# daijifeng001/MNC

Measured on NVIDIA H100. Metric: images/sec VGG16 MNC 5-stage @600x1000, 300 RoIs, higher is better.
Workload: dtype f16+2xf8 (fp16 main product + two e4m3 correction products on wgmma, fp32 accumulate, fp32-parity; conv1_1, K = 27: bf16x3)

## Files before the change

### mnc_b200/csrc/igemm_tc.cu

```cuda
#include <cuda.h>
#include <cuda_bf16.h>
#include <cuda_fp16.h>
#include <cuda_fp8.h>
#include <cuda_runtime.h>
#include <cstdint>
#include <cstdio>

#include "mnc_b200.h"
#include "ptx.cuh"
#include "tri.cuh"
#include "launch_util.h"

namespace mnc {

struct IgemmArgs {
  int batch, H, W;
  int Cin, Cout;
  int taps;
  int tiles_h, tiles_w, tiles_n;
  int k_steps;
  int split_k;
  int relu;
  int out_mode;
  const float* bias;
  __nv_bfloat16* out_hi;
  __nv_bfloat16* out_lo;
  uint8_t* out_x;
  float* out_f32;
  float acc_scale;
  float out_scale;
  unsigned int* amax;
  long long out_pix_stride;
  int out_ch_offset;
  long long split_stride;
  int vec_ok;
  int tma_store;
};

constexpr int kBlockM = 128;
constexpr int kBlockK = 64;
constexpr int kSmemMax = 227 * 1024;

constexpr int kXchgStride = 33;
constexpr int kXchgBytes = 2 * 128 * kXchgStride * 4;
constexpr int kStagingBytes = 2 * 2 * 128 * 64;
constexpr int kBarrierBytes = 1024;

template <int BN>
struct IgemmCfg {
  static constexpr int kABytes = kBlockM * kBlockK * 2;
  static constexpr int kBBytes = BN * kBlockK * 2;
  static constexpr int kStageBytes = 2 * kABytes + 2 * kBBytes;
  static constexpr int kFixedBytes = 1024  + kBarrierBytes + kXchgBytes + kStagingBytes;
  static constexpr int kStagesRaw = (kSmemMax - kFixedBytes) / kStageBytes;
  static constexpr int kStages = kStagesRaw > 8 ? 8 : kStagesRaw;
  static constexpr int kSmemBytes = kStages * kStageBytes + kFixedBytes;
  static_assert(kStages >= 2, "the ring needs two stages");
};

struct Tile {
  int img, h0, w0, n0, ks;
  int kb, kn, kstride;
};

__device__ __forceinline__ Tile decode_tile(const IgemmArgs& p, int t, int TH, int TW, int BN) {
  const int per_img = p.tiles_h * p.tiles_w;
  const int spatial = p.batch * per_img;
  const int sp = t % spatial;
  const int rest = t / spatial;
  const int nt = rest % p.tiles_n;
  Tile tl;
  tl.ks = rest / p.tiles_n;
  tl.img = sp / per_img;
  const int r = sp % per_img;
  tl.h0 = (r / p.tiles_w) * TH;
  tl.w0 = (r % p.tiles_w) * TW;
  tl.n0 = nt * BN;
  tl.kb = tl.ks;
  tl.kstride = p.split_k;
  tl.kn = (p.k_steps - tl.ks + p.split_k - 1) / p.split_k;
  return tl;
}


struct EpiState {
  int chunk_ctr;
  float amx;
};

template <int TH, int TW, int BN>
__device__ __forceinline__ void epilogue_tile(const IgemmArgs& p, const CUtensorMap* tm_o_hi_p,
                                              const CUtensorMap* tm_o_lo_p,
                                              const CUtensorMap* tm_o_x_p, float* xchg,
                                              uint8_t* staging, float (&acc)[BN / 64][32],
                                              const Tile& tl, int grp, EpiState& st) {
  const int tid = threadIdx.x & 127;
  const int lane = threadIdx.x & 31;
  constexpr int NBUF = 1;
  const int lead = 128 + grp * 128;
  const int row = tid;
  int& chunk_ctr = st.chunk_ctr;
  float& amx = st.amx;
  const float asc = p.acc_scale;
  const int img = tl.img, h0 = tl.h0, w0 = tl.w0, n0 = tl.n0, ks = tl.ks;
  const int h = h0 + row / TW;
  const int w = w0 + row % TW;
  const bool valid = (h < p.H) && (w < p.W);
  const long long pix = (static_cast<long long>(img) * p.H + h) * p.W + w;
  const int frow = grp * 64 + (tid >> 5) * 16 + (lane >> 2);
  const int fcol = (lane & 3) * 2;
#pragma unroll
  for (int nb = 0; nb < BN / 64; ++nb) {
    const int c0 = nb * 64 + grp * 32;
    uint32_t r[32];
    {
#pragma unroll
      for (int j = 0; j < 8; ++j) {
        const int col = j * 8 + fcol;
        float* d0 = xchg + ((col >> 5) * 128 + frow) * kXchgStride + (col & 31);
        d0[0] = acc[nb][4 * j];
        d0[1] = acc[nb][4 * j + 1];
        d0[8 * kXchgStride] = acc[nb][4 * j + 2];
        d0[8 * kXchgStride + 1] = acc[nb][4 * j + 3];
      }
      ptx::named_bar_sync(1, 256);
      const float* s0 = xchg + (grp * 128 + row) * kXchgStride;
#pragma unroll
      for (int j = 0; j < 32; ++j) r[j] = __float_as_uint(s0[j]);
      ptx::named_bar_sync(2, 256);
    }
      const int ch0 = n0 + c0;
      if (p.out_mode == 3) continue;
      if (p.out_mode == 2 || p.out_mode == 5) {
        const bool odd_x = (lane & 1) != 0;
        const bool odd_y = ((lane / TW) & 1) != 0;
        const int part = (odd_x ? 2 : 0) | (odd_y ? 1 : 0);
        const int hl = (row / TW) & ~1;
        const int wl = (row % TW) & ~1;
        float x[32];
#pragma unroll
        for (int j = 0; j < 32; ++j) x[j] = __uint_as_float(r[j]);
        if (!__all_sync(0xffffffffu, valid)) {
#pragma unroll
          for (int j = 0; j < 32; ++j) x[j] = valid ? x[j] : -3.402823466e+38f;
        }
        float y[16], m[8];
#pragma unroll
        for (int j = 0; j < 16; ++j) {
          const float keep = odd_x ? x[j + 16] : x[j];
          const float send = odd_x ? x[j] : x[j + 16];
          y[j] = fmaxf(keep, __shfl_xor_sync(0xffffffffu, send, 1));
        }
#pragma unroll
        for (int j = 0; j < 8; ++j) {
          const float keep = odd_y ? y[j + 8] : y[j];
          const float send = odd_y ? y[j] : y[j + 8];
          m[j] = fmaxf(keep, __shfl_xor_sync(0xffffffffu, send, TW));
        }
        const int hp = (h0 + hl) >> 1;
        const int wp = (w0 + wl) >> 1;
        const int Ho = (p.H + 1) >> 1, Wo = (p.W + 1) >> 1;
        const int chp = ch0 + part * 8;
        if (hp < Ho && wp < Wo && (h0 + hl) < p.H && (w0 + wl) < p.W &&
            chp < p.Cout) {
          const long long ppix = (static_cast<long long>(img) * Ho + hp) * Wo + wp;
          const long long poff = ppix * p.out_pix_stride + p.out_ch_offset + chp;
          float bv[8];
          if (p.bias != nullptr && chp + 8 <= p.Cout && (reinterpret_cast<uintptr_t>(p.bias + chp) & 15) == 0) {
            const float4 b0 = __ldg(reinterpret_cast<const float4*>(p.bias + chp));
            const float4 b1 = __ldg(reinterpret_cast<const float4*>(p.bias + chp) + 1);
            bv[0] = b0.x, bv[1] = b0.y, bv[2] = b0.z, bv[3] = b0.w;
            bv[4] = b1.x, bv[5] = b1.y, bv[6] = b1.z, bv[7] = b1.w;
          } else {
#pragma unroll
            for (int j = 0; j < 8; ++j)
              bv[j] = (p.bias != nullptr && chp + j < p.Cout) ? __ldg(p.bias + chp + j) : 0.f;
          }
#pragma unroll
          for (int j = 0; j < 8; ++j) {
            m[j] = m[j] * asc + bv[j];
            if (p.relu) m[j] = fmaxf(m[j], 0.f);
            if (chp + j < p.Cout) amx = fmaxf(amx, fabsf(m[j]));
          }
          if (p.out_mode == 5) {
            uint32_t hw[4], lw[2], cw[2];
#pragma unroll
            for (int e = 0; e < 4; ++e) {
              const Tri2 tr = tri_pack2(m[2 * e], m[2 * e + 1], p.out_scale);
              hw[e] = tr.h;
              if (e & 1) {
                lw[e >> 1] |= static_cast<uint32_t>(tr.l) << 16;
                cw[e >> 1] |= static_cast<uint32_t>(tr.c) << 16;
              } else {
                lw[e >> 1] = tr.l;
                cw[e >> 1] = tr.c;
              }
            }
            *reinterpret_cast<uint4*>(reinterpret_cast<__half*>(p.out_hi) + poff) =
                make_uint4(hw[0], hw[1], hw[2], hw[3]);
            *reinterpret_cast<uint2*>(reinterpret_cast<uint8_t*>(p.out_lo) + poff) = make_uint2(lw[0], lw[1]);
            *reinterpret_cast<uint2*>(p.out_x + poff) = make_uint2(cw[0], cw[1]);
            continue;
          }
          __nv_bfloat16* ph = p.out_hi + poff;
          __nv_bfloat16* pl = p.out_lo + poff;
          uint32_t hw[4], lw[4];
#pragma unroll
          for (int e = 0; e < 4; ++e) {
            const float x0 = m[2 * e], x1 = m[2 * e + 1];
            const __nv_bfloat16 h0b = __float2bfloat16_rn(x0);
            const __nv_bfloat16 h1b = __float2bfloat16_rn(x1);
            const __nv_bfloat16 l0b = __float2bfloat16_rn(x0 - __bfloat162float(h0b));
            const __nv_bfloat16 l1b = __float2bfloat16_rn(x1 - __bfloat162float(h1b));
            hw[e] = static_cast<uint32_t>(__bfloat16_as_ushort(h0b)) |
                    (static_cast<uint32_t>(__bfloat16_as_ushort(h1b)) << 16);
            lw[e] = static_cast<uint32_t>(__bfloat16_as_ushort(l0b)) |
                    (static_cast<uint32_t>(__bfloat16_as_ushort(l1b)) << 16);
          }
          *reinterpret_cast<uint4*>(ph) = make_uint4(hw[0], hw[1], hw[2], hw[3]);
          *reinterpret_cast<uint4*>(pl) = make_uint4(lw[0], lw[1], lw[2], lw[3]);
        }
      } else if (p.tma_store) {
        const bool tri = (p.out_mode == 4);
        const int buf = chunk_ctr % NBUF;
        uint8_t* sb = staging + (grp * NBUF + buf) * (2 * 128 * 64);
        if (threadIdx.x == lead) ptx::tma_store_wait_read<NBUF - 1>();
        ptx::named_bar_sync(3 + grp, 128);
        if (ch0 < p.Cout) {
          float bv[32];
          if (p.bias != nullptr && ch0 + 32 <= p.Cout &&
              (reinterpret_cast<uintptr_t>(p.bias + ch0) & 15) == 0) {
#pragma unroll
            for (int j4 = 0; j4 < 8; ++j4) {
              const float4 b4 = __ldg(reinterpret_cast<const float4*>(p.bias + ch0) + j4);
              bv[4 * j4] = b4.x;
              bv[4 * j4 + 1] = b4.y;
              bv[4 * j4 + 2] = b4.z;
              bv[4 * j4 + 3] = b4.w;
            }
          } else {
#pragma unroll
            for (int j = 0; j < 32; ++j)
              bv[j] = (p.bias != nullptr && ch0 + j < p.Cout) ? __ldg(p.bias + ch0 + j) : 0.f;
          }
          float mx = 0.f;
#pragma unroll
          for (int g = 0; g < 4; ++g) {
            uint32_t hw[4], lw[4];
#pragma unroll
            for (int e = 0; e < 4; ++e) {
              float x0 = __uint_as_float(r[g * 8 + 2 * e]) * asc + bv[g * 8 + 2 * e];
              float x1 = __uint_as_float(r[g * 8 + 2 * e + 1]) * asc + bv[g * 8 + 2 * e + 1];
              if (p.relu) {
                x0 = fmaxf(x0, 0.f);
                x1 = fmaxf(x1, 0.f);
              }
              mx = fmaxf(mx, fmaxf(fabsf(x0), fabsf(x1)));
              if (tri) {
                const Tri2 tr = tri_pack2(x0, x1, p.out_scale);
                hw[e] = tr.h;
                if (e & 1) {
                  lw[e >> 1] |= static_cast<uint32_t>(tr.l) << 16;
                  lw[2 + (e >> 1)] |= static_cast<uint32_t>(tr.c) << 16;
                } else {
                  lw[e >> 1] = tr.l;
                  lw[2 + (e >> 1)] = tr.c;
                }
              } else {
                const __nv_bfloat162 hp = __floats2bfloat162_rn(x0, x1);
                const uint32_t hbits = *reinterpret_cast<const uint32_t*>(&hp);
                const float f0 = __uint_as_float(hbits << 16);
                const float f1 = __uint_as_float(hbits & 0xffff0000u);
                const __nv_bfloat162 lp = __floats2bfloat162_rn(x0 - f0, x1 - f1);
                hw[e] = hbits;
                lw[e] = *reinterpret_cast<const uint32_t*>(&lp);
              }
            }
            const int off = row * 64 + ((g ^ ((row >> 1) & 3)) << 4);
            *reinterpret_cast<uint4*>(sb + off) = make_uint4(hw[0], hw[1], hw[2], hw[3]);
            if (tri) {
              *reinterpret_cast<uint2*>(sb + 128 * 64 + row * 32 + g * 8) = make_uint2(lw[0], lw[1]);
              *reinterpret_cast<uint2*>(sb + 128 * 96 + row * 32 + g * 8) = make_uint2(lw[2], lw[3]);
            } else {
              *reinterpret_cast<uint4*>(sb + 128 * 64 + off) = make_uint4(lw[0], lw[1], lw[2], lw[3]);
            }
          }
          if (valid) amx = fmaxf(amx, mx);
        }
        ptx::fence_proxy_async();
        ptx::named_bar_sync(3 + grp, 128);
        if (threadIdx.x == lead && ch0 < p.Cout) {
          ptx::tma_store_4d(tm_o_hi_p, sb, ch0, w0, h0, img);
          ptx::tma_store_4d(tm_o_lo_p, sb + 128 * 64, ch0, w0, h0, img);
          if (tri) ptx::tma_store_4d(tm_o_x_p, sb + 128 * 96, ch0, w0, h0, img);
          ptx::tma_store_commit();
        }
        ++chunk_ctr;
      } else if (valid && ch0 < p.Cout) {
        float v[32];
#pragma unroll
        for (int j = 0; j < 32; ++j) {
          float x = __uint_as_float(r[j]) * asc;
          if (p.bias != nullptr && ch0 + j < p.Cout) x += __ldg(p.bias + ch0 + j);
          if (p.relu) x = fmaxf(x, 0.f);
          v[j] = x;
          if (ch0 + j < p.Cout) amx = fmaxf(amx, fabsf(x));
        }
        const bool fullchunk = (ch0 + 32 <= p.Cout) && p.vec_ok;
        if (p.out_mode == 0) {
          __nv_bfloat16* ph = p.out_hi + pix * p.out_pix_stride + p.out_ch_offset + ch0;
          __nv_bfloat16* pl = p.out_lo + pix * p.out_pix_stride + p.out_ch_offset + ch0;
          if (fullchunk) {
#pragma unroll
            for (int g = 0; g < 4; ++g) {
              uint32_t hw[4], lw[4];
#pragma unroll
              for (int e = 0; e < 4; ++e) {
                const float x0 = v[g * 8 + 2 * e], x1 = v[g * 8 + 2 * e + 1];
                const __nv_bfloat16 h0b = __float2bfloat16_rn(x0);
                const __nv_bfloat16 h1b = __float2bfloat16_rn(x1);
                const __nv_bfloat16 l0b = __float2bfloat16_rn(x0 - __bfloat162float(h0b));
                const __nv_bfloat16 l1b = __float2bfloat16_rn(x1 - __bfloat162float(h1b));
                hw[e] = static_cast<uint32_t>(__bfloat16_as_ushort(h0b)) |
                        (static_cast<uint32_t>(__bfloat16_as_ushort(h1b)) << 16);
                lw[e] = static_cast<uint32_t>(__bfloat16_as_ushort(l0b)) |
                        (static_cast<uint32_t>(__bfloat16_as_ushort(l1b)) << 16);
              }
              *reinterpret_cast<uint4*>(ph + g * 8) = make_uint4(hw[0], hw[1], hw[2], hw[3]);
              *reinterpret_cast<uint4*>(pl + g * 8) = make_uint4(lw[0], lw[1], lw[2], lw[3]);
            }
          } else {
            for (int j = 0; j < 32 && ch0 + j < p.Cout; ++j) {
              const __nv_bfloat16 hb = __float2bfloat16_rn(v[j]);
              ph[j] = hb;
              pl[j] = __float2bfloat16_rn(v[j] - __bfloat162float(hb));
            }
          }
        } else {
          float* po = p.out_f32 + ks * p.split_stride + pix * p.out_pix_stride +
                      p.out_ch_offset + ch0;
          if (fullchunk) {
#pragma unroll
            for (int g = 0; g < 8; ++g)
              *reinterpret_cast<float4*>(po + g * 4) =
                  make_float4(v[g * 4], v[g * 4 + 1], v[g * 4 + 2], v[g * 4 + 3]);
          } else {
            for (int j = 0; j < 32 && ch0 + j < p.Cout; ++j) po[j] = v[j];
          }
        }
      }
  }
}

__device__ __forceinline__ void epilogue_finish(const IgemmArgs& p, int grp, const EpiState& st) {
  if (threadIdx.x == 128 + grp * 128) ptx::tma_store_wait_read<0>();
  if (p.amax != nullptr) {
    float amx = st.amx;
#pragma unroll
    for (int o = 16; o > 0; o >>= 1) amx = fmaxf(amx, __shfl_xor_sync(0xffffffffu, amx, o));
    if ((threadIdx.x & 31) == 0 && amx > 0.f) atomicMax(p.amax, __float_as_uint(amx));
  }
}

template <int TH, int TW, int BN, int PM>
__global__ void __launch_bounds__(384, 1)
igemm_tc_kernel(const __grid_constant__ CUtensorMap tm_a_hi, const __grid_constant__ CUtensorMap tm_a_lo,
                const __grid_constant__ CUtensorMap tm_a_x,
                const __grid_constant__ CUtensorMap tm_b_hi, const __grid_constant__ CUtensorMap tm_b_lo,
                const __grid_constant__ CUtensorMap tm_b_x,
                const __grid_constant__ CUtensorMap tm_o_hi, const __grid_constant__ CUtensorMap tm_o_lo,
                const __grid_constant__ CUtensorMap tm_o_x,
                const IgemmArgs p) {
  static_assert(TH * TW == kBlockM, "pixel tile must have 128 rows");
  using Cfg = IgemmCfg<BN>;
  constexpr int kStages = Cfg::kStages;
  constexpr int kABytes = Cfg::kABytes;
  constexpr int kBBytes = Cfg::kBBytes;
  constexpr int NB = BN / 64;

  extern __shared__ uint8_t smem_raw[];
  uint8_t* smem = reinterpret_cast<uint8_t*>((reinterpret_cast<uintptr_t>(smem_raw) + 1023) &
                                             ~static_cast<uintptr_t>(1023));
  uint64_t* full_bar = reinterpret_cast<uint64_t*>(smem + kStages * Cfg::kStageBytes);
  uint64_t* empty_bar = full_bar + kStages;
  uint8_t* staging = smem + kStages * Cfg::kStageBytes + kBarrierBytes;
  float* xchg = reinterpret_cast<float*>(staging + kStagingBytes);

  const int warp = threadIdx.x >> 5;
  const int lane = threadIdx.x & 31;
  const int wg = threadIdx.x >> 7;
  const int total_tiles = p.split_k * p.tiles_n * p.batch * p.tiles_h * p.tiles_w;
  const int kchunks = p.Cin / kBlockK;
  const int first = blockIdx.x;
  const int stride = gridDim.x;

  if (warp == 0 && lane == 0) {
    ptx::prefetch_tmap(&tm_a_hi);
    ptx::prefetch_tmap(&tm_a_lo);
    ptx::prefetch_tmap(&tm_b_hi);
    ptx::prefetch_tmap(&tm_b_lo);
    if (PM == 1) {
      ptx::prefetch_tmap(&tm_a_x);
      ptx::prefetch_tmap(&tm_b_x);
    }
  }
  if (warp == 1 && lane == 0) {
    for (int s = 0; s < kStages; ++s) {
      ptx::mbar_init(&full_bar[s], 1);
      ptx::mbar_init(&empty_bar[s], 2);
    }
    ptx::fence_barrier_init();
  }
  __syncthreads();

  if (wg == 0) {
    ptx::setmaxnreg_dec<40>();
    if (warp == 0) {
      int stage = 0;
      uint32_t phase = 0;
      constexpr int kNP = (PM == 0) ? 2 : 3;
      const CUtensorMap* amaps[3] = {&tm_a_hi, &tm_a_lo, &tm_a_x};
      const CUtensorMap* bmaps[3] = {&tm_b_hi, &tm_b_lo, &tm_b_x};
      for (int t = first; t < total_tiles; t += stride) {
        const Tile tl = decode_tile(p, t, TH, TW, BN);
        for (int i = 0, k = tl.kb; i < tl.kn; ++i, k += tl.kstride) {
          ptx::mbar_wait(&empty_bar[stage], phase ^ 1);
          uint8_t* st = smem + stage * Cfg::kStageBytes;
          ptx::mbar_arrive_expect_tx_w(&full_bar[stage], Cfg::kStageBytes);
          const int tap = k / kchunks;
          const int kc = k - tap * kchunks;
          int dy = 0, dx = 0;
          if (p.taps == 9) {
            dy = tap / 3 - 1;
            dx = tap % 3 - 1;
          }
#pragma unroll
          for (int pl = 0; pl < kNP; ++pl) {
            const int aoff = (PM == 0) ? pl * kABytes : (pl == 0 ? 0 : kABytes + (pl - 1) * (kABytes / 2));
            const int boff = (PM == 0) ? pl * kBBytes : (pl == 0 ? 0 : kBBytes + (pl - 1) * (kBBytes / 2));
            ptx::tma_load_4d_w(st + aoff, amaps[pl], &full_bar[stage], kc * kBlockK, tl.w0 + dx,
                               tl.h0 + dy, tl.img);
            ptx::tma_load_2d_w(st + 2 * kABytes + boff, bmaps[pl], &full_bar[stage],
                               tap * p.Cin + kc * kBlockK, tl.n0);
          }
          if (++stage == kStages) {
            stage = 0;
            phase ^= 1;
          }
        }
      }
    }
  } else {
    ptx::setmaxnreg_inc<232>();
    const int grp = wg - 1;
    const int tid = threadIdx.x & 127;
    float acc[NB][32];
    float accc[PM == 1 ? NB : 1][32];
    EpiState est = {0, 0.f};
    int stage = 0;
    uint32_t phase = 0;
    for (int t = first; t < total_tiles; t += stride) {
      const Tile tl = decode_tile(p, t, TH, TW, BN);
      for (int i = 0; i < tl.kn; ++i) {
        ptx::mbar_wait(&full_bar[stage], phase);
        const uint32_t a_hi = ptx::smem_u32(smem + stage * Cfg::kStageBytes) + grp * (kABytes / 2);
        const uint32_t b_hi = ptx::smem_u32(smem + stage * Cfg::kStageBytes) + 2 * kABytes;
#pragma unroll
        for (int nb = 0; nb < NB; ++nb) {
          ptx::wgmma_fence_acc(acc[nb]);
          if (PM == 1) ptx::wgmma_fence_acc(accc[nb]);
        }
        ptx::wgmma_fence();
        if (PM == 0) {
          const uint32_t a_lo = a_hi + kABytes;
          const uint32_t b_lo = b_hi + kBBytes;
#pragma unroll
          for (int kk = 0; kk < kBlockK / 16; ++kk) {
            const uint64_t da_hi = ptx::wgmma_desc_rows<128>(a_hi + kk * 32);
            const uint64_t da_lo = ptx::wgmma_desc_rows<128>(a_lo + kk * 32);
            const uint32_t acc0 = (i > 0 || kk > 0) ? 1u : 0u;
#pragma unroll
            for (int nb = 0; nb < NB; ++nb) {
              const uint64_t db_hi = ptx::wgmma_desc_rows<128>(b_hi + nb * (64 * 128) + kk * 32);
              const uint64_t db_lo = ptx::wgmma_desc_rows<128>(b_lo + nb * (64 * 128) + kk * 32);
              ptx::wgmma_bf16_n64(acc[nb], da_lo, db_hi, acc0);
              ptx::wgmma_bf16_n64(acc[nb], da_hi, db_lo, 1u);
              ptx::wgmma_bf16_n64(acc[nb], da_hi, db_hi, 1u);
            }
          }
        } else {
          const uint32_t a_l = ptx::smem_u32(smem + stage * Cfg::kStageBytes) + kABytes + grp * (kABytes / 4);
          const uint32_t a_c = a_l + kABytes / 2;
          const uint32_t b_c = b_hi + kBBytes, b_l = b_c + kBBytes / 2;
#pragma unroll
          for (int kk = 0; kk < kBlockK / 32; ++kk) {
            const uint64_t da_l = ptx::wgmma_desc_rows<64>(a_l + kk * 32);
            const uint64_t da_c = ptx::wgmma_desc_rows<64>(a_c + kk * 32);
            const uint32_t acc0 = (i > 0 || kk > 0) ? 1u : 0u;
#pragma unroll
            for (int nb = 0; nb < NB; ++nb) {
              const uint64_t db_c = ptx::wgmma_desc_rows<64>(b_c + nb * (64 * 64) + kk * 32);
              const uint64_t db_l = ptx::wgmma_desc_rows<64>(b_l + nb * (64 * 64) + kk * 32);
              ptx::wgmma_e4m3_n64(accc[nb], da_l, db_c, acc0);
              ptx::wgmma_e4m3_n64(accc[nb], da_c, db_l, 1u);
            }
          }
#pragma unroll
          for (int kk = 0; kk < kBlockK / 16; ++kk) {
            const uint64_t da = ptx::wgmma_desc_rows<128>(a_hi + kk * 32);
            const uint32_t acc0 = (i > 0 || kk > 0) ? 1u : 0u;
#pragma unroll
            for (int nb = 0; nb < NB; ++nb)
              ptx::wgmma_f16_n64(acc[nb], da, ptx::wgmma_desc_rows<128>(b_hi + nb * (64 * 128) + kk * 32), acc0);
          }
        }
        ptx::wgmma_commit();
        ptx::wgmma_wait_all();
#pragma unroll
        for (int nb = 0; nb < NB; ++nb) {
          ptx::wgmma_fence_acc(acc[nb]);
          if (PM == 1) ptx::wgmma_fence_acc(accc[nb]);
        }
        if (tid == 0) ptx::mbar_arrive(&empty_bar[stage]);
        if (++stage == kStages) {
          stage = 0;
          phase ^= 1;
        }
      }
      if (PM == 1) {
#pragma unroll
        for (int nb = 0; nb < NB; ++nb)
#pragma unroll
          for (int j = 0; j < 32; ++j) acc[nb][j] += accc[nb][j];
      }
      epilogue_tile<TH, TW, BN>(p, &tm_o_hi, &tm_o_lo, &tm_o_x, xchg, staging, acc, tl, grp, est);
    }
    epilogue_finish(p, grp, est);
  }
}

constexpr int kC11K = 32;
constexpr int kC11ABytes = kBlockM * kC11K * 2;
constexpr int kC11Stages = 2;
constexpr int kC11BBytes = 128 * kC11K * 2;
constexpr int kC11Ring = kC11Stages * 2 * kC11ABytes + kC11BBytes;
constexpr int kC11Smem = kC11Ring + kBarrierBytes + kStagingBytes + kXchgBytes + 1024 ;
constexpr int kC11Threads = 384;

__global__ void __launch_bounds__(kC11Threads, 1)
conv1_1_tc_kernel(const float* __restrict__ data, int B, int H, int W,
                  const __grid_constant__ CUtensorMap tm_b, const __grid_constant__ CUtensorMap tm_o_hi,
                  const __grid_constant__ CUtensorMap tm_o_lo, const __grid_constant__ CUtensorMap tm_o_x,
                  const IgemmArgs p) {
  constexpr int BN = 64;
  extern __shared__ uint8_t smem_raw[];
  uint8_t* smem = reinterpret_cast<uint8_t*>((reinterpret_cast<uintptr_t>(smem_raw) + 1023) &
                                             ~static_cast<uintptr_t>(1023));
  uint8_t* a_ring = smem;
  uint8_t* b_tile = smem + kC11Stages * 2 * kC11ABytes;
  uint64_t* a_full = reinterpret_cast<uint64_t*>(smem + kC11Ring);
  uint64_t* a_empty = a_full + kC11Stages;
  uint64_t* b_full = a_empty + kC11Stages;
  uint8_t* staging = smem + kC11Ring + kBarrierBytes;
  float* xchg = reinterpret_cast<float*>(staging + kStagingBytes);

  const int warp = threadIdx.x >> 5;
  const int lane = threadIdx.x & 31;
  const int wg = threadIdx.x >> 7;
  const int total_tiles = p.batch * p.tiles_w;
  const int first = blockIdx.x, stride = gridDim.x;

  if (warp == 0 && lane == 0) ptx::prefetch_tmap(&tm_b);
  if (warp == 1 && lane == 0) {
    for (int s = 0; s < kC11Stages; ++s) {
      ptx::mbar_init(&a_full[s], 128);
      ptx::mbar_init(&a_empty[s], 2);
    }
    ptx::mbar_init(b_full, 1);
    ptx::fence_barrier_init();
  }
  __syncthreads();

  if (wg == 0) {
    if (warp == 0) {
      ptx::mbar_arrive_expect_tx_w(b_full, kC11BBytes);
      ptx::tma_load_2d_w(b_tile, &tm_b, b_full, 0, 0);
    }
    const int pr = threadIdx.x;
    const long long plane = static_cast<long long>(H) * W;
    int as = 0;
    uint32_t aph = 0;
    for (int t = first; t < total_tiles; t += stride) {
      const int img = t / p.tiles_w;
      const int w = (t - img * p.tiles_w) * 128 + pr;
      const int b = img / H, h = img - b * H;
      float v[27];
      const float* xb = data + static_cast<long long>(b) * 3 * plane;
#pragma unroll
      for (int c = 0; c < 3; ++c)
#pragma unroll
        for (int ky = 0; ky < 3; ++ky)
#pragma unroll
          for (int kx = 0; kx < 3; ++kx) {
            const int hh = h + ky - 1, ww = w + kx - 1;
            const bool ok = hh >= 0 && hh < H && ww >= 0 && ww < W && w < W;
            v[c * 9 + ky * 3 + kx] = ok ? __ldg(xb + c * plane + static_cast<long long>(hh) * W + ww) : 0.f;
          }
      uint32_t hw[16], lw[16];
#pragma unroll
      for (int e = 0; e < 16; ++e) {
        const float x0 = (2 * e < 27) ? v[2 * e] : 0.f;
        const float x1 = (2 * e + 1 < 27) ? v[(2 * e + 1 < 27) ? 2 * e + 1 : 0] : 0.f;
        const __nv_bfloat16 h0 = __float2bfloat16_rn(x0), h1 = __float2bfloat16_rn(x1);
        const __nv_bfloat16 l0 = __float2bfloat16_rn(x0 - __bfloat162float(h0));
        const __nv_bfloat16 l1 = __float2bfloat16_rn(x1 - __bfloat162float(h1));
        hw[e] = static_cast<uint32_t>(__bfloat16_as_ushort(h0)) |
                (static_cast<uint32_t>(__bfloat16_as_ushort(h1)) << 16);
        lw[e] = static_cast<uint32_t>(__bfloat16_as_ushort(l0)) |
                (static_cast<uint32_t>(__bfloat16_as_ushort(l1)) << 16);
      }
      ptx::mbar_wait(&a_empty[as], aph ^ 1);
      uint8_t* sa = a_ring + as * 2 * kC11ABytes;
#pragma unroll
      for (int g = 0; g < 4; ++g) {
        const int off = pr * 64 + ((g ^ ((pr >> 1) & 3)) << 4);
        *reinterpret_cast<uint4*>(sa + off) = make_uint4(hw[4 * g], hw[4 * g + 1], hw[4 * g + 2], hw[4 * g + 3]);
        *reinterpret_cast<uint4*>(sa + kC11ABytes + off) =
            make_uint4(lw[4 * g], lw[4 * g + 1], lw[4 * g + 2], lw[4 * g + 3]);
      }
      ptx::fence_proxy_async();
      ptx::mbar_arrive(&a_full[as]);
      if (++as == kC11Stages) {
        as = 0;
        aph ^= 1;
      }
    }
  } else {
    const int grp = wg - 1;
    const int tid = threadIdx.x & 127;
    float acc[1][32];
    EpiState est = {0, 0.f};
    ptx::mbar_wait(b_full, 0);
    const uint32_t b_hi = ptx::smem_u32(b_tile);
    const uint32_t b_lo = b_hi + 64 * (kC11K * 2);
    int as = 0;
    uint32_t aph = 0;
    for (int t = first; t < total_tiles; t += stride) {
      const Tile tl = decode_tile(p, t, 1, 128, BN);
      ptx::mbar_wait(&a_full[as], aph);
      const uint32_t a_hi = ptx::smem_u32(a_ring + as * 2 * kC11ABytes) + grp * (kC11ABytes / 2);
      const uint32_t a_lo = a_hi + kC11ABytes;
      ptx::wgmma_fence_acc(acc[0]);
      ptx::wgmma_fence();
#pragma unroll
      for (int kk = 0; kk < kC11K / 16; ++kk) {
        const uint64_t da_hi = ptx::wgmma_desc_rows<64>(a_hi + kk * 32);
        const uint64_t da_lo = ptx::wgmma_desc_rows<64>(a_lo + kk * 32);
        const uint64_t db_hi = ptx::wgmma_desc_rows<64>(b_hi + kk * 32);
        const uint64_t db_lo = ptx::wgmma_desc_rows<64>(b_lo + kk * 32);
        ptx::wgmma_bf16_n64(acc[0], da_lo, db_hi, kk > 0 ? 1u : 0u);
        ptx::wgmma_bf16_n64(acc[0], da_hi, db_lo, 1u);
        ptx::wgmma_bf16_n64(acc[0], da_hi, db_hi, 1u);
      }
      ptx::wgmma_commit();
      ptx::wgmma_wait_all();
      ptx::wgmma_fence_acc(acc[0]);
      if (tid == 0) ptx::mbar_arrive(&a_empty[as]);
      if (++as == kC11Stages) {
        as = 0;
        aph ^= 1;
      }
      epilogue_tile<1, 128, BN>(p, &tm_o_hi, &tm_o_lo, &tm_o_x, xchg, staging, acc, tl, grp, est);
    }
    epilogue_finish(p, grp, est);
  }
}

typedef CUresult (*EncodeTiledFn)(CUtensorMap*, CUtensorMapDataType, cuuint32_t, void*,
                                  const cuuint64_t*, const cuuint64_t*, const cuuint32_t*,
                                  const cuuint32_t*, CUtensorMapInterleave, CUtensorMapSwizzle,
                                  CUtensorMapL2promotion, CUtensorMapFloatOOBfill);

static EncodeTiledFn get_encode_fn() {
  static EncodeTiledFn fn = nullptr;
  if (fn == nullptr) {
    void* ptr = nullptr;
    cudaDriverEntryPointQueryResult qres;
    if (cudaGetDriverEntryPoint("cuTensorMapEncodeTiled", &ptr, cudaEnableDefault, &qres) !=
            cudaSuccess ||
        qres != cudaDriverEntryPointSuccess) {
      return nullptr;
    }
    fn = reinterpret_cast<EncodeTiledFn>(ptr);
  }
  return fn;
}

static CUtensorMapSwizzle swizzle_for_row(int row_bytes) {
  return row_bytes >= 128 ? CU_TENSOR_MAP_SWIZZLE_128B
                          : (row_bytes == 64 ? CU_TENSOR_MAP_SWIZZLE_64B : CU_TENSOR_MAP_SWIZZLE_32B);
}

static int make_act_map(CUtensorMap* m, const void* base, int N, int H, int W, int C, int TH,
                        int TW, int bk, int eb = 2) {
  EncodeTiledFn enc = get_encode_fn();
  if (!enc) return MNC_ERR_DRIVER;
  cuuint64_t dims[4] = {(cuuint64_t)C, (cuuint64_t)W, (cuuint64_t)H, (cuuint64_t)N};
  cuuint64_t strides[3] = {(cuuint64_t)C * eb, (cuuint64_t)W * C * eb, (cuuint64_t)H * W * C * eb};
  cuuint32_t box[4] = {(cuuint32_t)bk, (cuuint32_t)TW, (cuuint32_t)TH, 1};
  cuuint32_t estr[4] = {1, 1, 1, 1};
  CUresult r = enc(m, eb == 2 ? CU_TENSOR_MAP_DATA_TYPE_BFLOAT16 : CU_TENSOR_MAP_DATA_TYPE_UINT8, 4,
                   const_cast<void*>(base), dims, strides, box, estr, CU_TENSOR_MAP_INTERLEAVE_NONE,
                   swizzle_for_row(bk * eb), CU_TENSOR_MAP_L2_PROMOTION_L2_128B,
                   CU_TENSOR_MAP_FLOAT_OOB_FILL_NONE);
  return r == CUDA_SUCCESS ? MNC_OK : MNC_ERR_DRIVER;
}

static int make_wgt_map(CUtensorMap* m, const void* base, int Cout, long long Ktot, int box_rows,
                        int bk, int eb = 2) {
  EncodeTiledFn enc = get_encode_fn();
  if (!enc) return MNC_ERR_DRIVER;
  cuuint64_t dims[2] = {(cuuint64_t)Ktot, (cuuint64_t)Cout};
  cuuint64_t strides[1] = {(cuuint64_t)Ktot * eb};
  cuuint32_t box[2] = {(cuuint32_t)bk, (cuuint32_t)box_rows};
  cuuint32_t estr[2] = {1, 1};
  CUresult r = enc(m, eb == 2 ? CU_TENSOR_MAP_DATA_TYPE_BFLOAT16 : CU_TENSOR_MAP_DATA_TYPE_UINT8, 2,
                   const_cast<void*>(base), dims, strides, box, estr, CU_TENSOR_MAP_INTERLEAVE_NONE,
                   swizzle_for_row(bk * eb), CU_TENSOR_MAP_L2_PROMOTION_L2_256B,
                   CU_TENSOR_MAP_FLOAT_OOB_FILL_NONE);
  return r == CUDA_SUCCESS ? MNC_OK : MNC_ERR_DRIVER;
}

static int make_out_map(CUtensorMap* m, const void* base, int N, int H, int W, int Cout,
                        long long pix_stride, int TH, int TW, int eb = 2) {
  EncodeTiledFn enc = get_encode_fn();
  if (!enc) return MNC_ERR_DRIVER;
  cuuint64_t dims[4] = {(cuuint64_t)Cout, (cuuint64_t)W, (cuuint64_t)H, (cuuint64_t)N};
  cuuint64_t strides[3] = {(cuuint64_t)pix_stride * eb, (cuuint64_t)W * pix_stride * eb,
                           (cuuint64_t)H * W * pix_stride * eb};
  cuuint32_t box[4] = {32, (cuuint32_t)TW, (cuuint32_t)TH, 1};
  cuuint32_t estr[4] = {1, 1, 1, 1};
  CUresult r = enc(m, eb == 2 ? CU_TENSOR_MAP_DATA_TYPE_BFLOAT16 : CU_TENSOR_MAP_DATA_TYPE_UINT8, 4,
                   const_cast<void*>(base), dims, strides, box, estr, CU_TENSOR_MAP_INTERLEAVE_NONE,
                   eb == 2 ? CU_TENSOR_MAP_SWIZZLE_64B : CU_TENSOR_MAP_SWIZZLE_NONE,
                   CU_TENSOR_MAP_L2_PROMOTION_NONE, CU_TENSOR_MAP_FLOAT_OOB_FILL_NONE);
  return r == CUDA_SUCCESS ? MNC_OK : MNC_ERR_DRIVER;
}

static int sm_count() {
  static int n = 0;
  if (n == 0) {
    int dev = 0;
    cudaGetDevice(&dev);
    cudaDeviceGetAttribute(&n, cudaDevAttrMultiProcessorCount, dev);
  }
  return n;
}

struct Maps {
  CUtensorMap a[3], b[3], o[3];
};

template <int TH, int TW, int BN, int PM>
static int launch_igemm(const Maps& m, const IgemmArgs& a, int max_ctas, cudaStream_t stream) {
  using Cfg = IgemmCfg<BN>;
  auto kern = igemm_tc_kernel<TH, TW, BN, PM>;
  static SmemGrant grant;
  if (!ensure_dynamic_smem(kern, Cfg::kSmemBytes, grant)) return MNC_ERR_CUDA;
  const int total = a.split_k * a.tiles_n * a.batch * a.tiles_h * a.tiles_w;
  int grid = sm_count();
  if (max_ctas > 0 && max_ctas < grid) grid = max_ctas;
  if (total < grid) grid = total;
  kern<<<grid, 384, Cfg::kSmemBytes, stream>>>(m.a[0], m.a[1], m.a[2], m.b[0], m.b[1], m.b[2], m.o[0],
                                               m.o[1], m.o[2], a);
  return cudaGetLastError() == cudaSuccess ? MNC_OK : MNC_ERR_CUDA;
}

}

using namespace mnc;

extern "C" int mnc_igemm_tc2(int in_fmt, const void* a0, const void* a1, const void* a2, int batch,
                             int H, int W, int Cin, const void* w0, const void* w1, const void* w2,
                             int Cout, int taps, const float* bias, int relu, int out_mode,
                             void* out0, void* out1, void* out2, long long out_pix_stride,
                             int out_ch_offset, int split_k, long long split_stride, int bn,
                             int max_ctas, float acc_scale, float out_scale, unsigned int* amax,
                             void* stream_) {
  cudaStream_t stream = static_cast<cudaStream_t>(stream_);
  if (Cin % 64 != 0 || (taps != 1 && taps != 9) || batch <= 0 || H <= 0 || W <= 0 || Cout <= 0)
    return MNC_ERR_ARG;
  if (in_fmt != 0 && in_fmt != 1) return MNC_ERR_ARG;
  if (out_mode != 0 && out_mode != 1 && out_mode != 2 && out_mode != 3 && out_mode != 4 && out_mode != 5)
    return MNC_ERR_ARG;
  const bool tri_out = (out_mode == 4 || out_mode == 5);
  const bool pooled = (out_mode == 2 || out_mode == 5);
  if (split_k < 1) split_k = 1;
  if (split_k > 1 && out_mode != 1) return MNC_ERR_ARG;
  if (pooled && (taps != 9 || Cout % 8 != 0 || out_pix_stride % 8 != 0 || out_ch_offset % 8 != 0))
    return MNC_ERR_ARG;
  if (tri_out && (out_pix_stride % 16 != 0 || out_ch_offset % 16 != 0 ||
                  (reinterpret_cast<uintptr_t>(out0) | reinterpret_cast<uintptr_t>(out1) |
                   reinterpret_cast<uintptr_t>(out2)) % 16 != 0))
    return MNC_ERR_ARG;
  const bool conv = (taps == 9);
  if (bn != 0 && bn != 64 && bn != 128 && bn != 192 && bn != 256) return MNC_ERR_ARG;
  if (bn == 0) bn = (Cout <= 64) ? 64 : 128;
  if (bn > 128) bn = 128;
  const int TH = conv ? 8 : 1, TW = conv ? 16 : 128;
  const int bk = kBlockK;

  IgemmArgs a;
  a.batch = batch;
  a.H = H;
  a.W = W;
  a.Cin = Cin;
  a.Cout = Cout;
  a.taps = taps;
  a.tiles_h = (H + TH - 1) / TH;
  a.tiles_w = (W + TW - 1) / TW;
  a.tiles_n = (Cout + bn - 1) / bn;
  a.k_steps = taps * (Cin / bk);
  if (split_k > a.k_steps) split_k = a.k_steps;
  a.split_k = split_k;
  a.relu = relu;
// ... 136 lines not shown
```

### mnc_b200/csrc/ptx.cuh

```cuda
#pragma once
#include <cstdint>
#include <cuda_runtime.h>

namespace mnc {
namespace ptx {

__device__ __forceinline__ uint32_t smem_u32(const void* p) {
  return static_cast<uint32_t>(__cvta_generic_to_shared(p));
}

__device__ __forceinline__ void mbar_init(uint64_t* bar, uint32_t count) {
  asm volatile("mbarrier.init.shared::cta.b64 [%0], %1;" ::"r"(smem_u32(bar)), "r"(count));
}
__device__ __forceinline__ void fence_barrier_init() {
  asm volatile("fence.mbarrier_init.release.cluster;" ::: "memory");
}
__device__ __forceinline__ void fence_proxy_async() {
  asm volatile("fence.proxy.async.shared::cta;" ::: "memory");
}
__device__ __forceinline__ void mbar_arrive(uint64_t* bar) {
  asm volatile("mbarrier.arrive.shared::cta.b64 _, [%0];" ::"r"(smem_u32(bar)) : "memory");
}
__device__ __forceinline__ bool mbar_try_wait(uint64_t* bar, uint32_t parity) {
  uint32_t ok;
  asm volatile(
      "{\n\t.reg .pred p;\n\t"
      "mbarrier.try_wait.parity.shared::cta.b64 p, [%1], %2;\n\t"
      "selp.b32 %0, 1, 0, p;\n\t}"
      : "=r"(ok)
      : "r"(smem_u32(bar)), "r"(parity)
      : "memory");
  return ok != 0;
}
__device__ __forceinline__ void mbar_wait(uint64_t* bar, uint32_t parity) {
  while (!mbar_try_wait(bar, parity)) {
  }
}

__device__ __forceinline__ void prefetch_tmap(const void* tmap) {
  asm volatile("prefetch.tensormap [%0];" ::"l"(reinterpret_cast<uint64_t>(tmap)) : "memory");
}

__device__ __forceinline__ void tma_store_4d(const void* tmap, const void* smem_src, int c0, int c1,
                                             int c2, int c3) {
  asm volatile(
      "cp.async.bulk.tensor.4d.global.shared::cta.bulk_group [%0, {%2, %3, %4, %5}], [%1];"
      ::"l"(reinterpret_cast<uint64_t>(tmap)), "r"(smem_u32(smem_src)), "r"(c0), "r"(c1), "r"(c2), "r"(c3)
      : "memory");
}
__device__ __forceinline__ void tma_store_commit() {
  asm volatile("cp.async.bulk.commit_group;" ::: "memory");
}
template <int kPending>
__device__ __forceinline__ void tma_store_wait_read() {
  asm volatile("cp.async.bulk.wait_group.read %0;" ::"n"(kPending) : "memory");
}
__device__ __forceinline__ void named_bar_sync(int id, int nthreads) {
  asm volatile("bar.sync %0, %1;" ::"r"(id), "r"(nthreads) : "memory");
}

__device__ __forceinline__ void mbar_arrive_expect_tx_w(uint64_t* bar, uint32_t bytes) {
  asm volatile(
      "{\n\t.reg .pred q;\n\t"
      "elect.sync _|q, 0xffffffff;\n\t"
      "@q mbarrier.arrive.expect_tx.shared::cta.b64 _, [%0], %1;\n\t}" ::"r"(smem_u32(bar)),
      "r"(bytes)
      : "memory");
}
__device__ __forceinline__ void tma_load_4d_w(void* smem_dst, const void* tmap, uint64_t* bar,
                                              int c0, int c1, int c2, int c3) {
  asm volatile(
      "{\n\t.reg .pred q;\n\t"
      "elect.sync _|q, 0xffffffff;\n\t"
      "@q cp.async.bulk.tensor.4d.shared::cluster.global.mbarrier::complete_tx::bytes"
      " [%0], [%1, {%3, %4, %5, %6}], [%2];\n\t}"
      ::"r"(smem_u32(smem_dst)),
      "l"(reinterpret_cast<uint64_t>(tmap)), "r"(smem_u32(bar)), "r"(c0), "r"(c1), "r"(c2), "r"(c3)
      : "memory");
}
__device__ __forceinline__ void tma_load_2d_w(void* smem_dst, const void* tmap, uint64_t* bar,
                                              int c0, int c1) {
  asm volatile(
      "{\n\t.reg .pred q;\n\t"
      "elect.sync _|q, 0xffffffff;\n\t"
      "@q cp.async.bulk.tensor.2d.shared::cluster.global.mbarrier::complete_tx::bytes"
      " [%0], [%1, {%3, %4}], [%2];\n\t}"
      ::"r"(smem_u32(smem_dst)),
      "l"(reinterpret_cast<uint64_t>(tmap)), "r"(smem_u32(bar)), "r"(c0), "r"(c1)
      : "memory");
}

template <int kRegs>
__device__ __forceinline__ void setmaxnreg_dec() {
  asm volatile("setmaxnreg.dec.sync.aligned.u32 %0;" ::"n"(kRegs));
}
template <int kRegs>
__device__ __forceinline__ void setmaxnreg_inc() {
  asm volatile("setmaxnreg.inc.sync.aligned.u32 %0;" ::"n"(kRegs));
}

template <int kRowBytes>
__device__ __forceinline__ uint64_t wgmma_desc_rows(uint32_t smem_addr) {
  static_assert(kRowBytes == 128 || kRowBytes == 64 || kRowBytes == 32, "row width");
  constexpr uint64_t kMode = kRowBytes == 128 ? 1 : (kRowBytes == 64 ? 2 : 3);
  uint64_t d = 0;
  d |= static_cast<uint64_t>((smem_addr & 0x3FFFFu) >> 4);
  d |= static_cast<uint64_t>(1) << 16;
  d |= static_cast<uint64_t>((8u * kRowBytes) >> 4) << 32;
  d |= kMode << 62;
  return d;
}

__device__ __forceinline__ void wgmma_fence() {
  asm volatile("wgmma.fence.sync.aligned;" ::: "memory");
}
__device__ __forceinline__ void wgmma_commit() {
  asm volatile("wgmma.commit_group.sync.aligned;" ::: "memory");
}
__device__ __forceinline__ void wgmma_wait_all() {
  asm volatile("wgmma.wait_group.sync.aligned 0;" ::: "memory");
}
__device__ __forceinline__ void wgmma_fence_acc(float (&d)[32]) {
#pragma unroll
  for (int j = 0; j < 32; ++j) asm volatile("" : "+f"(d[j])::"memory");
}

#define MNC_WGMMA_D32                                                                          \
  "{%0, %1, %2, %3, %4, %5, %6, %7, %8, %9, %10, %11, %12, %13, %14, %15, "                    \
  "%16, %17, %18, %19, %20, %21, %22, %23, %24, %25, %26, %27, %28, %29, %30, %31}"
#define MNC_WGMMA_D32_OPS(d)                                                                   \
  "+f"(d[0]), "+f"(d[1]), "+f"(d[2]), "+f"(d[3]), "+f"(d[4]), "+f"(d[5]), "+f"(d[6]),          \
      "+f"(d[7]), "+f"(d[8]), "+f"(d[9]), "+f"(d[10]), "+f"(d[11]), "+f"(d[12]), "+f"(d[13]),  \
      "+f"(d[14]), "+f"(d[15]), "+f"(d[16]), "+f"(d[17]), "+f"(d[18]), "+f"(d[19]),            \
      "+f"(d[20]), "+f"(d[21]), "+f"(d[22]), "+f"(d[23]), "+f"(d[24]), "+f"(d[25]),            \
      "+f"(d[26]), "+f"(d[27]), "+f"(d[28]), "+f"(d[29]), "+f"(d[30]), "+f"(d[31])

__device__ __forceinline__ void wgmma_bf16_n64(float (&d)[32], uint64_t desc_a, uint64_t desc_b,
                                               uint32_t accumulate) {
  asm volatile(
      "{\n\t.reg .pred p;\n\t"
      "setp.ne.b32 p, %34, 0;\n\t"
      "wgmma.mma_async.sync.aligned.m64n64k16.f32.bf16.bf16 " MNC_WGMMA_D32
      ", %32, %33, p, 1, 1, 0, 0;\n\t}"
      : MNC_WGMMA_D32_OPS(d)
      : "l"(desc_a), "l"(desc_b), "r"(accumulate));
}
__device__ __forceinline__ void wgmma_f16_n64(float (&d)[32], uint64_t desc_a, uint64_t desc_b,
                                              uint32_t accumulate) {
  asm volatile(
      "{\n\t.reg .pred p;\n\t"
      "setp.ne.b32 p, %34, 0;\n\t"
      "wgmma.mma_async.sync.aligned.m64n64k16.f32.f16.f16 " MNC_WGMMA_D32
      ", %32, %33, p, 1, 1, 0, 0;\n\t}"
      : MNC_WGMMA_D32_OPS(d)
      : "l"(desc_a), "l"(desc_b), "r"(accumulate));
}
__device__ __forceinline__ void wgmma_e4m3_n64(float (&d)[32], uint64_t desc_a, uint64_t desc_b,
                                               uint32_t accumulate) {
  asm volatile(
      "{\n\t.reg .pred p;\n\t"
      "setp.ne.b32 p, %34, 0;\n\t"
      "wgmma.mma_async.sync.aligned.m64n64k32.f32.e4m3.e4m3 " MNC_WGMMA_D32
      ", %32, %33, p, 1, 1;\n\t}"
      : MNC_WGMMA_D32_OPS(d)
      : "l"(desc_a), "l"(desc_b), "r"(accumulate));
}
#undef MNC_WGMMA_D32
#undef MNC_WGMMA_D32_OPS

}
}
```

Baseline: 276.6.

## Keep one wgmma group in flight and use n128 MMAs with stage-aliased exchange

The consumer loop now waits with wait_group 1 instead of draining all wgmma groups each k-step, releasing the previous stage only once its group has retired. This overlaps tensor-core work with the barrier and issue overhead. BN=128 tiles now issue one m64n128 wgmma instead of two n64 ones. The epilogue exchange buffer is moved out of fixed shared memory into the last consumed operand stage, freeing space for more pipeline stages. This adds cross-proxy fences and an extra barrier arrive, and it assumes the B layout for n128 is contiguous across both 64-column halves.

```diff
diff --git a/mnc_b200/csrc/igemm_tc.cu b/mnc_b200/csrc/igemm_tc.cu
--- a/mnc_b200/csrc/igemm_tc.cu
+++ b/mnc_b200/csrc/igemm_tc.cu
@@ -51,11 +51,14 @@
   static constexpr int kABytes = kBlockM * kBlockK * 2;
   static constexpr int kBBytes = BN * kBlockK * 2;
   static constexpr int kStageBytes = 2 * kABytes + 2 * kBBytes;
-  static constexpr int kFixedBytes = 1024  + kBarrierBytes + kXchgBytes + kStagingBytes;
+  static constexpr int kFixedBytes = 1024  + kBarrierBytes + kStagingBytes;
   static constexpr int kStagesRaw = (kSmemMax - kFixedBytes) / kStageBytes;
   static constexpr int kStages = kStagesRaw > 8 ? 8 : kStagesRaw;
   static constexpr int kSmemBytes = kStages * kStageBytes + kFixedBytes;
-  static_assert(kStages >= 2, "the ring needs two stages");
+  static_assert(kStages >= 3, "one group in flight plus one stage being filled needs three stages");
+  static_assert(kXchgBytes <= kStageBytes, "the epilogue exchange must fit in one operand stage");
+  static_assert(kSmemBytes <= kSmemMax, "shared memory beyond the opt-in limit");
+  static_assert(2 * kStages * 8 <= kBarrierBytes, "barrier area");
 };
 
 struct Tile {
@@ -92,7 +95,8 @@
 __device__ __forceinline__ void epilogue_tile(const IgemmArgs& p, const CUtensorMap* tm_o_hi_p,
                                               const CUtensorMap* tm_o_lo_p,
                                               const CUtensorMap* tm_o_x_p, float* xchg,
-                                              uint8_t* staging, float (&acc)[BN / 64][32],
+                                              uint64_t* xchg_empty, uint8_t* staging,
+                                              float (&acc)[BN / 64][32],
                                               const Tile& tl, int grp, EpiState& st) {
   const int tid = threadIdx.x & 127;
   const int lane = threadIdx.x & 31;
@@ -127,7 +131,10 @@
       const float* s0 = xchg + (grp * 128 + row) * kXchgStride;
 #pragma unroll
       for (int j = 0; j < 32; ++j) r[j] = __float_as_uint(s0[j]);
+      const bool last = (nb == BN / 64 - 1) && xchg_empty != nullptr;
+      if (last) ptx::fence_proxy_async();
       ptx::named_bar_sync(2, 256);
+      if (last && tid == 0) ptx::mbar_arrive(xchg_empty);
     }
       const int ch0 = n0 + c0;
       if (p.out_mode == 3) continue;
@@ -362,6 +369,22 @@
   }
 }
 
+template <int NB>
+__device__ __forceinline__ void mma_bf16(float (&d)[NB][32], uint64_t a, uint64_t b, uint32_t accum) {
+  if constexpr (NB == 2) ptx::wgmma_bf16_n128(d, a, b, accum);
+  else ptx::wgmma_bf16_n64(d[0], a, b, accum);
+}
+template <int NB>
+__device__ __forceinline__ void mma_f16(float (&d)[NB][32], uint64_t a, uint64_t b, uint32_t accum) {
+  if constexpr (NB == 2) ptx::wgmma_f16_n128(d, a, b, accum);
+  else ptx::wgmma_f16_n64(d[0], a, b, accum);
+}
+template <int NB>
+__device__ __forceinline__ void mma_e4m3(float (&d)[NB][32], uint64_t a, uint64_t b, uint32_t accum) {
+  if constexpr (NB == 2) ptx::wgmma_e4m3_n128(d, a, b, accum);
+  else ptx::wgmma_e4m3_n64(d[0], a, b, accum);
+}
+
 template <int TH, int TW, int BN, int PM>
 __global__ void __launch_bounds__(384, 1)
 igemm_tc_kernel(const __grid_constant__ CUtensorMap tm_a_hi, const __grid_constant__ CUtensorMap tm_a_lo,
@@ -372,6 +395,7 @@
                 const __grid_constant__ CUtensorMap tm_o_x,
                 const IgemmArgs p) {
   static_assert(TH * TW == kBlockM, "pixel tile must have 128 rows");
+  static_assert(BN == 64 || BN == 128, "one wgmma spans the tile: n64 or n128");
   using Cfg = IgemmCfg<BN>;
   constexpr int kStages = Cfg::kStages;
   constexpr int kABytes = Cfg::kABytes;
@@ -384,7 +408,6 @@
   uint64_t* full_bar = reinterpret_cast<uint64_t*>(smem + kStages * Cfg::kStageBytes);
   uint64_t* empty_bar = full_bar + kStages;
   uint8_t* staging = smem + kStages * Cfg::kStageBytes + kBarrierBytes;
-  float* xchg = reinterpret_cast<float*>(staging + kStagingBytes);
 
   const int warp = threadIdx.x >> 5;
   const int lane = threadIdx.x & 31;
@@ -461,6 +484,7 @@
     uint32_t phase = 0;
     for (int t = first; t < total_tiles; t += stride) {
       const Tile tl = decode_tile(p, t, TH, TW, BN);
+      int prev = 0;
       for (int i = 0; i < tl.kn; ++i) {
         ptx::mbar_wait(&full_bar[stage], phase);
         const uint32_t a_hi = ptx::smem_u32(smem + stage * Cfg::kStageBytes) + grp * (kABytes / 2);
@@ -471,22 +495,19 @@
           if (PM == 1) ptx::wgmma_fence_acc(accc[nb]);
         }
         ptx::wgmma_fence();
-        if (PM == 0) {
+        if constexpr (PM == 0) {
           const uint32_t a_lo = a_hi + kABytes;
           const uint32_t b_lo = b_hi + kBBytes;
 #pragma unroll
           for (int kk = 0; kk < kBlockK / 16; ++kk) {
             const uint64_t da_hi = ptx::wgmma_desc_rows<128>(a_hi + kk * 32);
             const uint64_t da_lo = ptx::wgmma_desc_rows<128>(a_lo + kk * 32);
+            const uint64_t db_hi = ptx::wgmma_desc_rows<128>(b_hi + kk * 32);
+            const uint64_t db_lo = ptx::wgmma_desc_rows<128>(b_lo + kk * 32);
             const uint32_t acc0 = (i > 0 || kk > 0) ? 1u : 0u;
-#pragma unroll
-            for (int nb = 0; nb < NB; ++nb) {
-              const uint64_t db_hi = ptx::wgmma_desc_rows<128>(b_hi + nb * (64 * 128) + kk * 32);
-              const uint64_t db_lo = ptx::wgmma_desc_rows<128>(b_lo + nb * (64 * 128) + kk * 32);
-              ptx::wgmma_bf16_n64(acc[nb], da_lo, db_hi, acc0);
-              ptx::wgmma_bf16_n64(acc[nb], da_hi, db_lo, 1u);
-              ptx::wgmma_bf16_n64(acc[nb], da_hi, db_hi, 1u);
-            }
+            mma_bf16<NB>(acc, da_lo, db_hi, acc0);
+            mma_bf16<NB>(acc, da_hi, db_lo, 1u);
+            mma_bf16<NB>(acc, da_hi, db_hi, 1u);
           }
         } else {
           const uint32_t a_l = ptx::smem_u32(smem + stage * Cfg::kStageBytes) + kABytes + grp * (kABytes / 4);
@@ -497,43 +518,48 @@
             const uint64_t da_l = ptx::wgmma_desc_rows<64>(a_l + kk * 32);
             const uint64_t da_c = ptx::wgmma_desc_rows<64>(a_c + kk * 32);
             const uint32_t acc0 = (i > 0 || kk > 0) ? 1u : 0u;
-#pragma unroll
-            for (int nb = 0; nb < NB; ++nb) {
-              const uint64_t db_c = ptx::wgmma_desc_rows<64>(b_c + nb * (64 * 64) + kk * 32);
-              const uint64_t db_l = ptx::wgmma_desc_rows<64>(b_l + nb * (64 * 64) + kk * 32);
-              ptx::wgmma_e4m3_n64(accc[nb], da_l, db_c, acc0);
-              ptx::wgmma_e4m3_n64(accc[nb], da_c, db_l, 1u);
-            }
+            mma_e4m3<NB>(accc, da_l, ptx::wgmma_desc_rows<64>(b_c + kk * 32), acc0);
+            mma_e4m3<NB>(accc, da_c, ptx::wgmma_desc_rows<64>(b_l + kk * 32), 1u);
           }
 #pragma unroll
           for (int kk = 0; kk < kBlockK / 16; ++kk) {
             const uint64_t da = ptx::wgmma_desc_rows<128>(a_hi + kk * 32);
             const uint32_t acc0 = (i > 0 || kk > 0) ? 1u : 0u;
-#pragma unroll
-            for (int nb = 0; nb < NB; ++nb)
-              ptx::wgmma_f16_n64(acc[nb], da, ptx::wgmma_desc_rows<128>(b_hi + nb * (64 * 128) + kk * 32), acc0);
+            mma_f16<NB>(acc, da, ptx::wgmma_desc_rows<128>(b_hi + kk * 32), acc0);
           }
         }
         ptx::wgmma_commit();
-        ptx::wgmma_wait_all();
-#pragma unroll
-        for (int nb = 0; nb < NB; ++nb) {
-          ptx::wgmma_fence_acc(acc[nb]);
-          if (PM == 1) ptx::wgmma_fence_acc(accc[nb]);
-        }
-        if (tid == 0) ptx::mbar_arrive(&empty_bar[stage]);
+        if (i > 0) {
+          ptx::wgmma_wait<1>();
+#pragma unroll
+          for (int nb = 0; nb < NB; ++nb) {
+            ptx::wgmma_fence_acc(acc[nb]);
+            if (PM == 1) ptx::wgmma_fence_acc(accc[nb]);
+          }
+          if (tid == 0) ptx::mbar_arrive(&empty_bar[prev]);
+        }
+        prev = stage;
         if (++stage == kStages) {
           stage = 0;
           phase ^= 1;
         }
       }
+      ptx::wgmma_wait<0>();
+#pragma unroll
+      for (int nb = 0; nb < NB; ++nb) {
+        ptx::wgmma_fence_acc(acc[nb]);
+        if (PM == 1) ptx::wgmma_fence_acc(accc[nb]);
+      }
       if (PM == 1) {
 #pragma unroll
         for (int nb = 0; nb < NB; ++nb)
 #pragma unroll
           for (int j = 0; j < 32; ++j) acc[nb][j] += accc[nb][j];
       }
-      epilogue_tile<TH, TW, BN>(p, &tm_o_hi, &tm_o_lo, &tm_o_x, xchg, staging, acc, tl, grp, est);
+      ptx::named_bar_sync(1, 256);
+      epilogue_tile<TH, TW, BN>(p, &tm_o_hi, &tm_o_lo, &tm_o_x,
+                                reinterpret_cast<float*>(smem + prev * Cfg::kStageBytes), &empty_bar[prev],
+                                staging, acc, tl, grp, est);
     }
     epilogue_finish(p, grp, est);
   }
@@ -663,14 +689,14 @@
         ptx::wgmma_bf16_n64(acc[0], da_hi, db_hi, 1u);
       }
       ptx::wgmma_commit();
-      ptx::wgmma_wait_all();
+      ptx::wgmma_wait<0>();
       ptx::wgmma_fence_acc(acc[0]);
       if (tid == 0) ptx::mbar_arrive(&a_empty[as]);
       if (++as == kC11Stages) {
         as = 0;
         aph ^= 1;
       }
-      epilogue_tile<1, 128, BN>(p, &tm_o_hi, &tm_o_lo, &tm_o_x, xchg, staging, acc, tl, grp, est);
+      epilogue_tile<1, 128, BN>(p, &tm_o_hi, &tm_o_lo, &tm_o_x, xchg, nullptr, staging, acc, tl, grp, est);
     }
     epilogue_finish(p, grp, est);
   }
diff --git a/mnc_b200/csrc/ptx.cuh b/mnc_b200/csrc/ptx.cuh
--- a/mnc_b200/csrc/ptx.cuh
+++ b/mnc_b200/csrc/ptx.cuh
@@ -117,8 +117,9 @@
 __device__ __forceinline__ void wgmma_commit() {
   asm volatile("wgmma.commit_group.sync.aligned;" ::: "memory");
 }
-__device__ __forceinline__ void wgmma_wait_all() {
-  asm volatile("wgmma.wait_group.sync.aligned 0;" ::: "memory");
+template <int kPending>
+__device__ __forceinline__ void wgmma_wait() {
+  asm volatile("wgmma.wait_group.sync.aligned %0;" ::"n"(kPending) : "memory");
 }
 __device__ __forceinline__ void wgmma_fence_acc(float (&d)[32]) {
 #pragma unroll
@@ -165,6 +166,46 @@
       : MNC_WGMMA_D32_OPS(d)
       : "l"(desc_a), "l"(desc_b), "r"(accumulate));
 }
+
+#define MNC_WGMMA_D64                                                                          \
+  "{%0, %1, %2, %3, %4, %5, %6, %7, %8, %9, %10, %11, %12, %13, %14, %15, "                    \
+  "%16, %17, %18, %19, %20, %21, %22, %23, %24, %25, %26, %27, %28, %29, %30, %31, "           \
+  "%32, %33, %34, %35, %36, %37, %38, %39, %40, %41, %42, %43, %44, %45, %46, %47, "           \
+  "%48, %49, %50, %51, %52, %53, %54, %55, %56, %57, %58, %59, %60, %61, %62, %63}"
+#define MNC_WGMMA_D64_OPS(d) MNC_WGMMA_D32_OPS(d[0]), MNC_WGMMA_D32_OPS(d[1])
+
+__device__ __forceinline__ void wgmma_bf16_n128(float (&d)[2][32], uint64_t desc_a, uint64_t desc_b,
+                                                uint32_t accumulate) {
+  asm volatile(
+      "{\n\t.reg .pred p;\n\t"
+      "setp.ne.b32 p, %66, 0;\n\t"
+      "wgmma.mma_async.sync.aligned.m64n128k16.f32.bf16.bf16 " MNC_WGMMA_D64
+      ", %64, %65, p, 1, 1, 0, 0;\n\t}"
+      : MNC_WGMMA_D64_OPS(d)
+      : "l"(desc_a), "l"(desc_b), "r"(accumulate));
+}
+__device__ __forceinline__ void wgmma_f16_n128(float (&d)[2][32], uint64_t desc_a, uint64_t desc_b,
+                                               uint32_t accumulate) {
+  asm volatile(
+      "{\n\t.reg .pred p;\n\t"
+      "setp.ne.b32 p, %66, 0;\n\t"
+      "wgmma.mma_async.sync.aligned.m64n128k16.f32.f16.f16 " MNC_WGMMA_D64
+      ", %64, %65, p, 1, 1, 0, 0;\n\t}"
+      : MNC_WGMMA_D64_OPS(d)
+      : "l"(desc_a), "l"(desc_b), "r"(accumulate));
+}
+__device__ __forceinline__ void wgmma_e4m3_n128(float (&d)[2][32], uint64_t desc_a, uint64_t desc_b,
+                                                uint32_t accumulate) {
+  asm volatile(
+      "{\n\t.reg .pred p;\n\t"
+      "setp.ne.b32 p, %66, 0;\n\t"
+      "wgmma.mma_async.sync.aligned.m64n128k32.f32.e4m3.e4m3 " MNC_WGMMA_D64
+      ", %64, %65, p, 1, 1;\n\t}"
+      : MNC_WGMMA_D64_OPS(d)
+      : "l"(desc_a), "l"(desc_b), "r"(accumulate));
+}
+#undef MNC_WGMMA_D64
+#undef MNC_WGMMA_D64_OPS
 #undef MNC_WGMMA_D32
 #undef MNC_WGMMA_D32_OPS
 
```

After: 274.3 (median of 6 runs). No clear change (-0.8%).
